# phoenix163/JeicybooDSP

Measured on AMD Instinct MI355X. Metric: STFT frames/s (1024-pt, 50% OLA), higher is better.
Workload: dtype f32; 1 GPU; STFT analysis n_fft=1024 hop=512 Hamming, batch=65536 frames/GPU, int16 PCM in HBM -> complex64 full spectrum in HBM; frames_per_gpu=65536, parallelism=frame-sharded x1, no collective, launch=hipGraph replay of the K steps, pcm_buffers=6, pcm_bytes_total=402659328

## Files before the change

### jeicyboodsp_amd/csrc/fft_c2c_kernels.hip

```cpp
#include "jdsp_internal.h"

namespace jdsp {

__device__ __forceinline__ short bitrev16(int k, int bits, int n_fft)
{
    short walk = (short)k;
    short rev = walk;
    for (int i = 1; i < bits; i++) {
        walk = (short)(walk >> 1);
        rev = (short)(unsigned short)(((unsigned)(unsigned short)rev) << 1);
        rev = (short)(rev | (walk & 1));
    }
    return (short)(rev & (n_fft - 1));
}

__global__ void bitrev_table_kernel(short *table, int n_fft, int bits)
{
    const int k = blockIdx.x * blockDim.x + threadIdx.x;
    if (k < n_fft) table[k] = bitrev16(k, bits, n_fft);
}

__global__ __launch_bounds__(256) void fft_process_f64_kernel(const double2 *__restrict__ in, double2 *__restrict__ out,
                                                             int n_fft, int log2n, int forward,
                                                             const double2 *__restrict__ tw)
{
    extern __shared__ __attribute__((aligned(16))) char smem_raw[];
    double2 *x = reinterpret_cast<double2 *>(smem_raw);
    const double2 *src = in + (size_t)blockIdx.x * n_fft;
    double2 *dst = out + (size_t)blockIdx.x * n_fft;
    for (int k = threadIdx.x; k < n_fft; k += blockDim.x)
        x[(unsigned short)bitrev16(k, log2n, n_fft)] = src[k];
    __syncthreads();
    const int half_n = n_fft >> 1;
// ... 248 lines not shown
#pragma unroll
    for (int d = 0; d < 8; d++) {
        const cd zm = lds[512 - lane - 64 * d];
        const double2 w = wsp[64 * d];
        const cd e = {v[d].x + zm.x, v[d].y - zm.y};
        const cd o = {v[d].y + zm.y, zm.x - v[d].x};
        const cd p = cd_mul(o, cd{w.x, w.y});
        f64x2 lo = {0.5 * (e.x + p.x), 0.5 * (e.y + p.y)}, hi = {0.5 * (e.x - p.x), 0.5 * (e.y - p.y)};
        __builtin_nontemporal_store(lo, dst + 64 * d);
        __builtin_nontemporal_store(hi, dst + 64 * d + 512);
    }
    lds_fence_wave();
  }
}

__device__ __forceinline__ void cd_opaque(cd &a) { asm volatile("" : "+v"(a.x), "+v"(a.y)); }
__device__ __forceinline__ void cd_powers(const cd &b, cd (&p)[8])
{
    p[1] = b;
    p[2] = cd_mul(b, b);
    p[3] = cd_mul(p[2], b);
    p[4] = cd_mul(p[2], p[2]);
    p[5] = cd_mul(p[4], b);
    p[6] = cd_mul(p[3], p[3]);
    p[7] = cd_mul(p[4], p[3]);
}

#ifndef JDSP_F64_PLAIN_STORES
#define JDSP_F64_PLAIN_STORES 0
#endif
#ifndef JDSP_F64_LINEAR_MAP
#define JDSP_F64_LINEAR_MAP 1
#endif
template <bool DW, bool LOOP>
__global__ __launch_bounds__(64, (JDSP_F64_SWIZZLE && !LOOP) ? 5 : 4) void stft1024_f64_v2_kernel(const short *__restrict__ pcm, long n_frames, long hop,
                                                               const double *__restrict__ table,
                                                               const double2 *__restrict__ tw, double2 *__restrict__ out,
                                                               int run)
{
    constexpr bool SWZ = JDSP_F64_SWIZZLE && !LOOP;
    __shared__ __attribute__((aligned(16))) cd lds[SWZ ? 512 : kFft512Lds];
    const int lane = threadIdx.x;
#if JDSP_F64_LINEAR_MAP
    const long t0 = (long)blockIdx.x * run;
#else
    const long per_xcd = (gridDim.x + 7) >> 3;
    const long t0 = ((long)(blockIdx.x & 7) * per_xcd + (blockIdx.x >> 3)) * run;
#endif
    if (t0 >= n_frames) return;
    const long t1 = LOOP ? (t0 + run < n_frames ? t0 + run : n_frames) : t0 + 1;
    double2 win[8];
    {
        const double2 *wp = reinterpret_cast<const double2 *>(table) + lane;
#pragma unroll
        for (int r = 0; r < 8; r++) win[r] = wp[64 * r];
    }
    cd b1 = w512<false>(tw, lane), b2 = w512<false>(tw, 8 * (lane & 7));
    cd b3;
    {
        const double2 q = (reinterpret_cast<const double2 *>(table + 1024))[lane];
        b3 = {q.x, q.y};
    }
    unsigned int raw[8];
    short raw16[16];
    auto fetch = [&](long t) {
        const short *src = pcm + t * hop + 2 * lane;
        if (DW) {
#pragma unroll
            for (int r = 0; r < 8; r++) raw[r] = *reinterpret_cast<const unsigned int *>(src + 128 * r);
        } else {
#pragma unroll
            for (int r = 0; r < 8; r++) { raw16[2 * r] = src[128 * r]; raw16[2 * r + 1] = src[128 * r + 1]; }
        }
    };
    fetch(t0);
    unsigned int tk[8];
#pragma unroll
    for (int r = 0; r < 8; r++) tk[r] = raw[r];
#pragma unroll 1
    for (long t = t0; t < t1; t++) {
// ... 63 lines not shown
        for (int d = 0; d < 8; d++) lds[lane + 64 * d] = v[d];
        if constexpr (!SWZ) { if (lane == 0) lds[512] = v[0]; }
        lds_fence_wave();
        if (LOOP && DW && t + 1 < t1) {
#pragma unroll
            for (int r = 0; r < 8; r++) { tk[r] = raw[r]; asm volatile("" : "+v"(tk[r])); }
            __builtin_amdgcn_sched_barrier(0);
        }
        typedef double f64x2 __attribute__((ext_vector_type(2)));
        f64x2 *dst = reinterpret_cast<f64x2 *>(out + t * 1024 + lane);
        constexpr double c1 = 0.92387953251128675613, s1 = 0.38268343236508977173, h = 0.70710678118654752440;
        const cd w16[8] = {{1.0, 0.0}, {c1, -s1}, {h, -h}, {s1, -c1}, {0.0, -1.0}, {-s1, -c1}, {-h, -h}, {-c1, -s1}};
#pragma unroll
        for (int d = 0; d < 8; d++) {
            const cd zm = lds[SWZ ? ((512 - lane - 64 * d) & 511) : (512 - lane - 64 * d)];
            const cd w = d == 0 ? b3 : (d == 4 ? cd{b3.y, -b3.x} : cd_mul(b3, w16[d]));
            const cd e = {v[d].x + zm.x, v[d].y - zm.y};
            const cd o = {v[d].y + zm.y, zm.x - v[d].x};
            const cd pp = cd_mul(o, w);
            f64x2 lo = {0.5 * (e.x + pp.x), 0.5 * (e.y + pp.y)}, hi = {0.5 * (e.x - pp.x), 0.5 * (e.y - pp.y)};
#if JDSP_F64_PLAIN_STORES
            dst[64 * d] = lo;
            dst[64 * d + 512] = hi;
#else
            __builtin_nontemporal_store(lo, dst + 64 * d);
            __builtin_nontemporal_store(hi, dst + 64 * d + 512);
#endif
        }
        lds_fence_wave();
    }
}

int launch_stft1024_f64(hipStream_t stream, int n_cu, const short *pcm, long n_frames, long hop, const double *table,
                        const double2 *tw512, double2 *out, int variant, int fpw)
{
    if (n_frames <= 0) return 0;
    const long slots = 4096;
    const long run = fpw > 0 ? fpw : (variant == 1 ? (n_frames + slots - 1) / slots : 1);
    (void)n_cu;
    const long waves = (n_frames + run - 1) / run;
    const long grid = (waves + 7) / 8 * 8;
    if (variant == 1)
        hipLaunchKernelGGL(stft1024_f64_kernel, dim3((unsigned)grid), dim3(64), 0, stream, pcm, n_frames, hop, table, tw512,
                           out, (int)run);
    else {
        const bool dw = (((uintptr_t)pcm) & 3u) == 0 && (hop & 1) == 0;
#define JDSP_F64_LAUNCH(DW_, LOOP_) hipLaunchKernelGGL((stft1024_f64_v2_kernel<DW_, LOOP_>), dim3((unsigned)grid), dim3(64), 0, stream, pcm, \
                                                       n_frames, hop, table, tw512, out, (int)run)
        if (run > 1) { if (dw) JDSP_F64_LAUNCH(true, true); else JDSP_F64_LAUNCH(false, true); }
        else { if (dw) JDSP_F64_LAUNCH(true, false); else JDSP_F64_LAUNCH(false, false); }
#undef JDSP_F64_LAUNCH
    }
    return hipGetLastError() == hipSuccess ? 0 : -1;
}

void fill_stft1024_f64_table(double *t)
{
    const double PI = 3.141592;
    for (int i = 0; i < 1024; i++) t[i] = 0.54 - 0.46 * cos(2 * PI * i / (1024 - 1));
    const double two_pi = 6.283185307179586476925286766559;
    for (int m = 0; m < 512; m++) {
        const double a = -two_pi * (double)m / 1024.0;
        t[1024 + 2 * m] = cos(a);
        t[1024 + 2 * m + 1] = sin(a);
    }
}

int launch_fft_process_f64(hipStream_t stream, const double2 *in, double2 *out, int n_fft, int log2n, long batch,
                           int forward, const double2 *tw)
{
    if (batch <= 0) return 0;
    if (n_fft == 512 && (((uintptr_t)in | (uintptr_t)out) & 15u) == 0) {
        const long grid = (batch + 7) / 8 * 8;
        if (forward) hipLaunchKernelGGL(fft512_f64_kernel<false>, dim3((unsigned)grid), dim3(64), 0, stream, in, out, batch, tw);
        else hipLaunchKernelGGL(fft512_f64_kernel<true>, dim3((unsigned)grid), dim3(64), 0, stream, in, out, batch, tw);
        return hipGetLastError() == hipSuccess ? 0 : -1;
    }
    const size_t lds = sizeof(double2) * (size_t)n_fft;
    int threads = n_fft / 2 < 256 ? (n_fft / 2 < 64 ? 64 : n_fft / 2) : 256;
    if (lds > 64 * 1024) {
        hipError_t e = hipFuncSetAttribute((const void *)fft_process_f64_kernel,
                                           hipFuncAttributeMaxDynamicSharedMemorySize, (int)lds);
        if (e != hipSuccess) return -1;
    }
    hipLaunchKernelGGL(fft_process_f64_kernel, dim3((unsigned)batch), dim3(threads), lds, stream, in, out, n_fft, log2n,
                       forward, tw);
// ... 14 lines not shown
```

### jeicyboodsp_amd/csrc/jdsp_api.hip

```cpp
#include "jdsp_internal.h"

static std::string g_create_error;

namespace jdsp {

int fail(jdsp_ctx *ctx, int code, const char *what, hipError_t e)
{
    std::string msg = what ? what : "error";
    if (e != hipSuccess) {
        msg += ": ";
        msg += hipGetErrorString(e);
    }
    if (ctx) ctx->error = msg;
    else g_create_error = msg;
    return code;
}

static int ensure_stft1024_table_of(jdsp_ctx *ctx, DevBuf<float2> &table, int window_kind)
{
    return ensure_table(ctx, table, (size_t)stft1024_table_count(),
                        [window_kind](float2 *t) { fill_stft1024_table(t, window_kind); });
}

int ensure_stft1024_table(jdsp_ctx *ctx) { return ensure_stft1024_table_of(ctx, ctx->stft1024_table, 0); }

int ensure_stft1024_table_rect(jdsp_ctx *ctx) { return ensure_stft1024_table_of(ctx, ctx->stft1024_table_rect, 2); }

int ensure_vad_window(jdsp_ctx *ctx)
{
    return ensure_table(ctx, ctx->vad_w_hi, 512, [](double *w) {
        for (int i = 0; i < 512; i++) w[i] = (0.54 - 0.46 * cos(2 * 3.141592 * (512 + i) / (1024 - 1)));
    });
}
// ... 19 lines not shown

int jdsp_abi_version(void) { return JDSP_ABI_VERSION; }

int jdsp_create(int device, jdsp_ctx **out)
{
    if (!out) return fail(nullptr, JDSP_EINVAL, "jdsp_create: out is NULL");
    *out = nullptr;
    int count = 0;
    hipError_t e = hipGetDeviceCount(&count);
    if (e != hipSuccess || count <= 0)
        return fail(nullptr, JDSP_ENODEV, "jdsp_create: no HIP device (this library has no CPU fallback)", e);
    if (device < 0 || device >= count) return fail(nullptr, JDSP_ENODEV, "jdsp_create: device ordinal out of range");
    jdsp_ctx *ctx = new (std::nothrow) jdsp_ctx();
    if (!ctx) return fail(nullptr, JDSP_ENOMEM, "jdsp_create: out of host memory");
    ctx->device = device;
    hipDeviceProp_t prop;
    if ((e = hipSetDevice(device)) != hipSuccess || (e = hipGetDeviceProperties(&prop, device)) != hipSuccess) {
        delete ctx;
        return fail(nullptr, JDSP_EHIP, "jdsp_create: device query", e);
    }
    ctx->n_cu = prop.multiProcessorCount;
    ctx->hbm_bytes = prop.totalGlobalMem;
    snprintf(ctx->name, sizeof(ctx->name), "%s (%s)", prop.name, prop.gcnArchName);
    if (strncmp(prop.gcnArchName, "gfx950", 6) != 0) {
        std::string m = std::string("jdsp_create: device is ") + prop.gcnArchName + ", this library is built for gfx950 only";
        delete ctx;
        return fail(nullptr, JDSP_ENODEV, m.c_str());
    }
    if ((e = hipStreamCreateWithFlags(&ctx->own_stream, hipStreamNonBlocking)) != hipSuccess) {
        delete ctx;
        return fail(nullptr, JDSP_EHIP, "jdsp_create: hipStreamCreate", e);
    }
    ctx->stream = ctx->own_stream;
    *out = ctx;
    return JDSP_OK;
}

int jdsp_destroy(jdsp_ctx *ctx)
{
    if (!ctx) return JDSP_OK;
    (void)hipSetDevice(ctx->device);
    (void)hipStreamSynchronize(ctx->stream);
    const hipEvent_t events[] = {ctx->pipe_ev[0], ctx->pipe_ev[1], ctx->pipe_ev[2], ctx->pipe_ev[3],
                                 ctx->pipe_ev[4], ctx->pipe_ev[5], ctx->switch_ev};
    const hipStream_t streams[] = {ctx->pipe_in, ctx->pipe_out, ctx->own_stream};
    delete ctx;
    for (hipEvent_t ev : events)
        if (ev) (void)hipEventDestroy(ev);
    for (hipStream_t st : streams)
        if (st) (void)hipStreamDestroy(st);
    return JDSP_OK;
}

const char *jdsp_last_error(const jdsp_ctx *ctx) { return ctx ? ctx->error.c_str() : g_create_error.c_str(); }

static int switch_stream(jdsp_ctx *ctx, hipStream_t next)
{
    if (next == ctx->stream) return JDSP_OK;
    hipStreamCaptureStatus a = hipStreamCaptureStatusNone, b = hipStreamCaptureStatusNone;
    const bool ok_a = hipStreamIsCapturing(ctx->stream, &a) == hipSuccess;
    const bool ok_b = hipStreamIsCapturing(next, &b) == hipSuccess;
    if (!ok_a || !ok_b) (void)hipGetLastError();
    if (ok_a && ok_b && a == hipStreamCaptureStatusNone && b == hipStreamCaptureStatusNone) {
        JDSP_HIP(ctx, hipSetDevice(ctx->device));
        if (!ctx->switch_ev) JDSP_HIP(ctx, hipEventCreateWithFlags(&ctx->switch_ev, hipEventDisableTiming));
        JDSP_HIP(ctx, hipEventRecord(ctx->switch_ev, ctx->stream));
// ... 239 lines not shown
    float *d_max = hc.alloc<float>(n * 4);
    float *d_ac = autocorr_host ? hc.alloc<float>(n * 2048) : nullptr;
    if (hc.ok()) hc.result(jdsp_pitch_autocorr_dev(ctx, d_in, n_blocks, d_prev, d_arg, d_max, d_ac));
    hc.download(arg_host, d_arg, n * 4);
    hc.download(rmax_host, d_max, n * 4);
    hc.download(autocorr_host, d_ac, n * 2048);
    return hc.finish();
}

int jdsp_stft_i16_dev(jdsp_ctx *ctx, const int16_t *pcm_dev, long n_frames, int n_fft, int hop, jdsp_c32 *spec_dev)
{
    if (!ctx) return JDSP_EINVAL;
    if (n_fft != 1024 && n_fft != 512) return fail(ctx, JDSP_EINVAL, "jdsp_stft_i16_dev: n_fft must be 1024 or 512");
    if (hop < 1) return fail(ctx, JDSP_EINVAL, "jdsp_stft_i16_dev: hop must be >= 1");
    if (n_frames < 0 || (n_frames > 0 && (!pcm_dev || !spec_dev)))
        return fail(ctx, JDSP_EINVAL, "jdsp_stft_i16_dev: bad buffer");
    if (n_frames == 0) return JDSP_OK;
    if ((uintptr_t)pcm_dev & 1u) return fail(ctx, JDSP_EINVAL, "jdsp_stft_i16_dev: pcm must be 2-byte aligned");
    if ((uintptr_t)spec_dev & 15u) return fail(ctx, JDSP_EINVAL, "jdsp_stft_i16_dev: spec must be 16-byte aligned");
    JDSP_HIP(ctx, hipSetDevice(ctx->device));
    int rc = jdsp::ensure_stft1024_table(ctx);
    if (rc) return rc;
    const int wk = ctx->opt_stft_window;
    if (wk == 1 && (rc = jdsp::ensure_stft1024_table_of(ctx, ctx->stft1024_table_hann, 1))) return rc;
    const float2 *tab = wk == 1 ? ctx->stft1024_table_hann.get() : ctx->stft1024_table.get();
    if (n_fft == 512) {
        jdsp::DevBuf<float2> &w512 = wk == 1 ? ctx->win512_hann : ctx->win512;
        if ((rc = jdsp::ensure_table(ctx, w512, 256, [wk](float2 *w) { jdsp::fill_win512(w, wk); }))) return rc;
        if (jdsp::launch_stft512(ctx->stream, ctx->n_cu, pcm_dev, n_frames, hop, (float2 *)spec_dev, tab, w512.get()))
            return fail(ctx, JDSP_EHIP, "stft512 launch", hipGetLastError());
        return JDSP_OK;
    }
    if (jdsp::launch_stft1024(ctx->stream, ctx->n_cu, ctx->opt_stft_fpw, pcm_dev, n_frames, hop, (float2 *)spec_dev, tab,
                              ctx->opt_stft_read_pass, ctx->opt_stft_touch_wg))
        return fail(ctx, JDSP_EHIP, "stft1024 launch", hipGetLastError());
    return JDSP_OK;
}

int jdsp_stft_half_i16_dev(jdsp_ctx *ctx, const int16_t *pcm_dev, long n_frames, jdsp_c32 *spec_dev, long row_pitch)
{
    if (!ctx) return JDSP_EINVAL;
    if (n_frames < 0 || (n_frames > 0 && (!pcm_dev || !spec_dev))) return fail(ctx, JDSP_EINVAL, "jdsp_stft_half_i16_dev: bad buffer");
    if (row_pitch < 513) return fail(ctx, JDSP_EINVAL, "jdsp_stft_half_i16_dev: row_pitch must be at least 513");
    if (n_frames == 0) return JDSP_OK;
    if (((uintptr_t)pcm_dev & 15u) || ((uintptr_t)spec_dev & 15u))
        return fail(ctx, JDSP_EINVAL, "jdsp_stft_half_i16_dev: buffers must be 16-byte aligned");
    JDSP_HIP(ctx, hipSetDevice(ctx->device));
    int rc = jdsp::ensure_stft1024_table(ctx);
    if (rc) return rc;
    if (jdsp::launch_stft1024_half(ctx->stream, pcm_dev, n_frames, (float2 *)spec_dev, row_pitch, ctx->stft1024_table.get()))
        return fail(ctx, JDSP_EHIP, "stft half launch", hipGetLastError());
    return JDSP_OK;
}

static const char kStftBatchPitch[] =
    "jdsp_stft_half_batch: row_pitch must be even and >= 514 (every row 16-byte aligned: the even-row store)";

int jdsp_stft_half_batch_dev(jdsp_ctx *ctx, const int16_t *pcm_dev, const int64_t *sample_first_dev,
                             const int64_t *frame_first_dev, long n_utts, long n_frames_total, int hop, jdsp_c32 *spec_dev,
                             long row_pitch)
{
    if (!ctx) return JDSP_EINVAL;
    if (n_utts < 0 || n_frames_total < 0) return fail(ctx, JDSP_EINVAL, "jdsp_stft_half_batch: n_utts or n_frames_total < 0");
    if (hop != 1024 && hop != 512 && hop != 256)
        return fail(ctx, JDSP_EINVAL, "jdsp_stft_half_batch: hop must be 1024, 512 or 256 (n_fft, n_fft/2 or n_fft/4)");
    if (row_pitch < 514 || (row_pitch & 1)) return fail(ctx, JDSP_EINVAL, kStftBatchPitch);
    if (!jdsp::aligned(pcm_dev, 4) || !jdsp::aligned(spec_dev, 16) || !jdsp::aligned(sample_first_dev, 8) ||
// ... 62 lines not shown
        e = hipEventRecord(ev_comp[b], comp);
        if (e == hipSuccess) e = hipStreamWaitEvent(ctx->pipe_out, ev_comp[b], 0);
        if (e == hipSuccess) e = hipMemcpyAsync(spec_host + (size_t)f0 * n_fft, d_out, sizeof(jdsp_c32) * (size_t)nf * n_fft, hipMemcpyDeviceToHost, ctx->pipe_out);
        if (e == hipSuccess) e = hipEventRecord(ev_out[b], ctx->pipe_out);
        if (e != hipSuccess) rc = fail(ctx, JDSP_EHIP, "stft pipeline: copy out", e);
    }
    hipError_t e1 = hipStreamSynchronize(ctx->pipe_in), e2 = hipStreamSynchronize(comp), e3 = hipStreamSynchronize(ctx->pipe_out);
    if (!rc && (e1 != hipSuccess || e2 != hipSuccess || e3 != hipSuccess)) rc = fail(ctx, JDSP_EHIP, "stft pipeline: sync", e1 != hipSuccess ? e1 : (e2 != hipSuccess ? e2 : e3));
    return rc;
}

static int ensure_c2c_tw(jdsp_ctx *ctx, int n_fft, int lg)
{
    return jdsp::ensure_table(ctx, ctx->c2c_tw[lg], (size_t)n_fft / 2 + 1,
                              [n_fft](double2 *t) { jdsp::fill_c2c_twiddles(t, n_fft); });
}

int jdsp_stft_i16_f64_dev(jdsp_ctx *ctx, const int16_t *pcm_dev, long n_frames, int n_fft, int hop, double *spec_dev)
{
    if (!ctx) return JDSP_EINVAL;
    if (n_fft != 1024) return fail(ctx, JDSP_EINVAL, "jdsp_stft_i16_f64_dev: n_fft must be 1024");
    if (hop < 1) return fail(ctx, JDSP_EINVAL, "jdsp_stft_i16_f64_dev: hop must be >= 1");
    if (n_frames < 0 || (n_frames > 0 && (!pcm_dev || !spec_dev))) return fail(ctx, JDSP_EINVAL, "jdsp_stft_i16_f64_dev: bad buffer");
    if (n_frames == 0) return JDSP_OK;
    if ((uintptr_t)pcm_dev & 1u) return fail(ctx, JDSP_EINVAL, "jdsp_stft_i16_f64_dev: pcm must be 2-byte aligned");
    if ((uintptr_t)spec_dev & 15u) return fail(ctx, JDSP_EINVAL, "jdsp_stft_i16_f64_dev: spec must be 16-byte aligned");
    JDSP_HIP(ctx, hipSetDevice(ctx->device));
    int rc = ensure_c2c_tw(ctx, 512, 9);
    if (rc) return rc;
    if ((rc = jdsp::ensure_table(ctx, ctx->stft_f64_table, 1024 + 2 * 512, jdsp::fill_stft1024_f64_table))) return rc;
    const int rp = ctx->opt_stft_read_pass;
    const bool touch = hop == 512 && ((uintptr_t)pcm_dev & 15u) == 0 && (rp > 0 || (rp < 0 && n_frames >= 16384));
    const long slab = touch ? 65536 : n_frames;
    for (long f0 = 0; f0 < n_frames; f0 += slab) {
        const long nf = n_frames - f0 < slab ? n_frames - f0 : slab;
        if ((touch && jdsp::launch_pcm_read_pass(ctx->stream, ctx->n_cu, ctx->opt_stft_touch_wg, pcm_dev + f0 * hop, hop * (nf + 1))) ||
            jdsp::launch_stft1024_f64(ctx->stream, ctx->n_cu, pcm_dev + f0 * hop, nf, hop, ctx->stft_f64_table.get(), ctx->c2c_tw[9].get(),
                                      (double2 *)spec_dev + f0 * 1024, ctx->opt_stft_f64_kernel, ctx->opt_stft_f64_fpw)) {
            const hipError_t le = hipGetLastError();
            return fail(ctx, JDSP_EHIP, "stft f64 launch", le);
        }
    }
    return JDSP_OK;
}

int jdsp_stft_i16_f64(jdsp_ctx *ctx, const int16_t *pcm_host, long n_samples, int n_fft, int hop, double *spec_host,
                      long *n_frames_out)
{
    if (!ctx) return JDSP_EINVAL;
    if (n_fft != 1024 || hop < 1) return fail(ctx, JDSP_EINVAL, "jdsp_stft_i16_f64: unsupported n_fft/hop");
    const long n_frames = n_samples >= n_fft ? (n_samples - n_fft) / hop + 1 : 0;
    if (n_frames_out) *n_frames_out = n_frames;
    if (n_frames == 0) return JDSP_OK;
    if (!pcm_host || !spec_host) return fail(ctx, JDSP_EINVAL, "jdsp_stft_i16_f64: NULL buffer");
    JDSP_HIP(ctx, hipSetDevice(ctx->device));
    const size_t in_bytes = sizeof(int16_t) * (size_t)((n_frames - 1) * hop + n_fft);
    const size_t out_bytes = 2 * sizeof(double) * (size_t)n_frames * (size_t)n_fft;
    jdsp::HostCall hc(ctx, "jdsp_stft_i16_f64");
    const int16_t *d_in = hc.upload(pcm_host, in_bytes);
    double *d_out = hc.alloc<double>(out_bytes);
    if (hc.ok()) hc.result(jdsp_stft_i16_f64_dev(ctx, d_in, n_frames, n_fft, hop, d_out));
    hc.download(spec_host, d_out, out_bytes);
    return hc.finish();
}

int jdsp_stft_i16(jdsp_ctx *ctx, const int16_t *pcm_host, long n_samples, int n_fft, int hop, jdsp_c32 *spec_host,
                  long *n_frames_out)
{
    if (!ctx) return JDSP_EINVAL;
    if ((n_fft != 1024 && n_fft != 512) || hop < 1) return fail(ctx, JDSP_EINVAL, "jdsp_stft_i16: unsupported n_fft/hop");
    long n_frames = n_samples >= n_fft ? (n_samples - n_fft) / hop + 1 : 0;
// ... 51 lines not shown
```

### jeicyboodsp_amd/csrc/jdsp_internal.h

```cpp
#pragma once
#include <hip/hip_runtime.h>

#include <cmath>
#include <cstdlib>
#include <cstdint>
#include <cstdio>
#include <cstring>
#include <string>
#include <vector>

#include "../../include/jdsp.h"
#include "ragged_layout.h"

namespace jdsp {

template <class T> class DevBuf {
public:
    DevBuf() = default;
    DevBuf(DevBuf &&o) noexcept : p_(o.p_), n_(o.n_) { o.p_ = nullptr, o.n_ = 0; }
    DevBuf &operator=(DevBuf &&o) noexcept
    {
        if (this != &o) {
            reset();
            p_ = o.p_, n_ = o.n_;
// ... 16 lines not shown
        void *p = nullptr;
        const hipError_t e = hipMalloc(&p, count * sizeof(T));
        if (e == hipSuccess) p_ = (T *)p, n_ = count;
        return e;
    }
    hipError_t upload(const T *host, size_t count)
    {
        hipError_t e = alloc(count);
        if (e == hipSuccess && (e = hipMemcpy(p_, host, count * sizeof(T), hipMemcpyHostToDevice)) != hipSuccess) reset();
        return e;
    }
    hipError_t grow(size_t count) { return count <= n_ ? hipSuccess : alloc(count); }

private:
    T *p_ = nullptr;
    size_t n_ = 0;
};

}

struct jdsp_ctx {
    int device = 0;
    int n_cu = 0;
    size_t hbm_bytes = 0;
    char name[64] = {0};
    hipStream_t own_stream = nullptr;
    hipStream_t stream = nullptr;
    hipEvent_t switch_ev = nullptr;
    std::string error;
    int opt_stft_fpw = 0;
    int opt_stft_window = 0;
    int opt_stft_read_pass = -1;
    int opt_stft_touch_wg = 0;
    int opt_stft_f64_kernel = 0;
    int opt_stft_f64_fpw = 0;
    jdsp::DevBuf<float2> stft1024_table;
    jdsp::DevBuf<float2> stft1024_table_hann, win512_hann;
    jdsp::DevBuf<float2> stft1024_table_rect;
    jdsp::DevBuf<float2> win512;
    jdsp::DevBuf<double2> c2c_tw[16];
    jdsp::DevBuf<double> stft_f64_table;
    jdsp::DevBuf<float2> conv_tw4096, conv_tw8192;
    jdsp::DevBuf<double> vad_w_hi;
    jdsp::DevBuf<double> vad_w_ex[2][2];
    jdsp::DevBuf<double> lpc_win[2];
    hipStream_t pipe_in = nullptr, pipe_out = nullptr;
    hipEvent_t pipe_ev[6] = {nullptr, nullptr, nullptr, nullptr, nullptr, nullptr};
    jdsp::DevBuf<char> pipe_buf[4];
};

namespace jdsp {

struct DenoiseState {
    int run_len;
    int pad[3];
    float avg[1024];
    float noise[1024];
    short prev[512];
    float tail[512];
};
struct DenoisePlan { int n_events, n_snap, pad0, pad1; };

constexpr int kNoiseChunks = 4096;
struct NoiseAccum {
    float *chunk_alpha;
    float *chunk_beta;
// ... 143 lines not shown

template <class T, class Fill> int ensure_table(jdsp_ctx *ctx, DevBuf<T> &buf, size_t count, Fill fill)
{
    if (buf.get()) return JDSP_OK;
    std::vector<T> host(count);
    fill(host.data());
    const hipError_t e = buf.upload(host.data(), count);
    return e == hipSuccess ? JDSP_OK : fail(ctx, JDSP_EHIP, "device table", e);
}

struct RunPlanWs {
    DevBuf<unsigned char> flags;
    DevBuf<int> events, ev_n;
    DevBuf<int> ver_base;
    DevBuf<unsigned long long> snap_mask;
    long cap_blocks = 0;

    hipError_t reserve(size_t n)
    {
        hipError_t e = flags.alloc(n);
        if (e == hipSuccess) e = events.alloc(n);
        if (e == hipSuccess) e = ev_n.alloc(n);
        if (e == hipSuccess) e = ver_base.alloc(n / 64 + 1);
        if (e == hipSuccess) e = snap_mask.alloc(n / 64 + 1);
        if (e == hipSuccess) cap_blocks = (long)n;
        else *this = RunPlanWs();
        return e;
    }
};

int stft1024_table_count();
void fill_stft1024_table(float2 *host_table, int window_kind);
int launch_stft1024(hipStream_t stream, int n_cu, int fpw_opt, const short *pcm, long n_frames, long hop, float2 *spec,
                    const float2 *table, int read_pass = 0, int touch_wg_per_cu = 0);


int launch_stft1024_half(hipStream_t stream, const short *pcm, long n_frames, float2 *spec, long pitch,
                         const float2 *table);
int launch_stft512(hipStream_t stream, int n_cu, const short *pcm, long n_frames, long hop, float2 *spec,
                   const float2 *table, const float2 *win512);
void fill_win512(float2 *w, int window_kind);
int launch_stft_half_batch(hipStream_t s, int hop, int run_opt, const short *pcm, const long long *sample_first,
                           const long long *frame_first, long n_utts, long n_frames_total, float2 *spec, long pitch,
                           const float2 *table);

int launch_bitrev_table(hipStream_t stream, short *table_dev, int n_fft, int bits);
int launch_fft_process_f64(hipStream_t stream, const double2 *in, double2 *out, int n_fft, int log2n, long batch,
                           int forward, const double2 *tw);
void fill_c2c_twiddles(double2 *t, int n_fft);
int launch_stft1024_f64(hipStream_t stream, int n_cu, const short *pcm, long n_frames, long hop, const double *table,
                        const double2 *tw512, double2 *out, int variant, int fpw);
int launch_pcm_read_pass(hipStream_t stream, int n_cu, int wg_per_cu, const short *pcm, long n_samples);
void fill_stft1024_f64_table(double *t);
int launch_dft_direct_f64(hipStream_t stream, int kind, const void *in, double2 *inout, int n, long batch);


int launch_vad(hipStream_t s, int block_len, const short *pcm, long n_blocks, const double *w_hi, int use_zcr,
               unsigned char *flags, long long *dbg_energy, int *dbg_zcr);
int launch_run_plan(hipStream_t s, const unsigned char *flags, long n_blocks, const int *run_len_in, int *run_len_out,
                    int latch_run, int *ver_base, unsigned long long *snap_mask, int *events, int *ev_n,
                    DenoisePlan *plan);
int launch_denoise_plan(hipStream_t s, const unsigned char *flags, long n_blocks, const DenoiseState *st_in,
                        DenoiseState *st_out, int *ver_base, unsigned long long *snap_mask, int *events, int *ev_n,
                        DenoisePlan *plan);
int launch_noise_estimate(hipStream_t s, DenoiseGeom g, const short *pcm, long n_blocks, const DenoiseState *st_in,
                          DenoiseState *st_out, const int *events, const int *ev_n, const DenoisePlan *plan,
                          const int *ver_base, const unsigned long long *snap_mask, const float2 *table,
                          const NoiseAccum &acc, float *noise_rows);
int launch_denoise(hipStream_t s, DenoiseGeom g, int mode, int k_opt, int n_cu, const short *pcm, long n_blocks,
                   long calls_before, const DenoiseState *st_in, DenoiseState *st_out, const int *ver_base,
                   const unsigned long long *snap_mask, const float *noise_rows, const float2 *table, short *out,
                   float *precast, int *redo, const DenoiseShard *shard = nullptr);
int launch_shard_summary(hipStream_t s, DenoiseGeom g, const short *pcm_ext, long n_ext, long ext0, long b0, long b1,
                         const int *events, const int *ev_n, const DenoisePlan *plan, const int *ver_base,
                         const unsigned long long *snap_mask, const float2 *table, int *range, const NoiseAccum &acc,
                         float *rows, float *summary);
int launch_shard_rows(hipStream_t s, DenoiseGeom g, const float *summaries_all, int rank, long b0, long b1,
                      const DenoisePlan *plan, const int *range, const NoiseAccum &acc, float *a_in, float *rows,
                      float *last);
int launch_shard_row0(hipStream_t s, DenoiseGeom g, const float *last_all, int rank, float *rows);
int launch_denoise_batch(hipStream_t s, int mode, int run_opt, int n_cu, const short *pcm, const long long *sample_first,
                         const long long *block_first, long n_utts, long n_blocks, const double *w_hi,
                         const float2 *table, unsigned char *flags, int *row_idx, float *rows, int *redo, short *out,
                         float *precast, float *noise_last, int vad_only);
// ... 348 lines not shown
```

### jeicyboodsp_amd/csrc/stft_kernels.hip

```cpp
#include "frame_io.h"
#include "jdsp_internal.h"
#include "ola_stream.h"
#include "ragged_batch.h"

namespace jdsp {

#ifndef JDSP_STFT_K
#define JDSP_STFT_K 2
#endif
#ifndef JDSP_STFT_MINWAVES
#define JDSP_STFT_MINWAVES 4
#endif
#ifndef JDSP_STFT_XCD
#define JDSP_STFT_XCD 1
#endif
#ifndef JDSP_STFT_NT_LOAD
#define JDSP_STFT_NT_LOAD 0
#endif
#ifndef JDSP_STFT_NT
#define JDSP_STFT_NT 1
#endif
#ifndef JDSP_STFT_DIRECT
#define JDSP_STFT_DIRECT 1
#endif
#ifndef JDSP_STFT_ABLATE
#define JDSP_STFT_ABLATE 0
#endif

__device__ __forceinline__ void store_spec(float4 *p, float4 v)
{
#if JDSP_STFT_NT
    f32x4 t = {v.x, v.y, v.z, v.w};
    __builtin_nontemporal_store(t, reinterpret_cast<f32x4 *>(p));
#else
    *p = v;
#endif
}

template <int J>
__device__ __forceinline__ void split_store_j(const float2 *lds, int lane, const float2 *wsp, float4 *dst)
{
    const int m = 128 * J + 2 * lane;
    const float4 zz = *reinterpret_cast<const float4 *>(&lds[m]);
    float2 zr0, zr1;
    load_mirror_pair(lds, m, zr0, zr1);
    float2 lo0, hi0, lo1, hi1;
    split_fwd<J>(make_float2(zz.x, zz.y), zr0, wsp[0], lo0, hi0);
    split_fwd<J>(make_float2(zz.z, zz.w), zr1, wsp[1], lo1, hi1);
    store_spec(dst + 64 * J, make_float4(lo0.x, lo0.y, lo1.x, lo1.y));
    store_spec(dst + 64 * J + 256, make_float4(hi0.x, hi0.y, hi1.x, hi1.y));
}

__device__ __forceinline__ void split_and_store(const float2 *lds, int lane, const float2 *wsp, float2 *out_frame)
{
    float4 *dst = reinterpret_cast<float4 *>(out_frame) + lane;
    split_store_j<0>(lds, lane, wsp, dst);
    split_store_j<1>(lds, lane, wsp, dst);
    split_store_j<2>(lds, lane, wsp, dst);
    split_store_j<3>(lds, lane, wsp, dst);
}

template <int K>
__global__ __launch_bounds__(64, JDSP_STFT_MINWAVES) void stft1024_hop512_kernel(
    const short *__restrict__ pcm, float2 *__restrict__ spec, long n_frames, const float2 *__restrict__ table)
{
    __shared__ __attribute__((aligned(16))) float2 lds[kWaveLdsComplex];
    __shared__ __attribute__((aligned(16))) unsigned int stage[256];
    const int lane = threadIdx.x;
#if JDSP_STFT_XCD
    const long per_xcd = (gridDim.x + 7) >> 3;
    const long f0 = ((long)(blockIdx.x & 7) * per_xcd + (blockIdx.x >> 3)) * K;
#else
    const long f0 = (long)blockIdx.x * K;
#endif
    if (f0 >= n_frames) return;

#if JDSP_STFT_DIRECT
    const unsigned int *pcm32 = reinterpret_cast<const unsigned int *>(pcm) + lane;
    unsigned int half[K + 1][4];
#pragma unroll
    for (int h = 0; h <= K; h++) {
        const long hh = f0 + h <= n_frames ? f0 + h : n_frames;
#pragma unroll
        for (int q = 0; q < 4; q++) half[h][q] = pcm32[hh * 256 + 64 * q];
    }
#else
    const u32x4 *pcm128 = reinterpret_cast<const u32x4 *>(pcm) + lane;
    u32x4 half[K + 1];
#pragma unroll
    for (int h = 0; h <= K; h++) {
        const long hh = f0 + h <= n_frames ? f0 + h : n_frames;
#if JDSP_STFT_NT_LOAD
        half[h] = __builtin_nontemporal_load(pcm128 + hh * 64);
#else
        half[h] = pcm128[hh * 64];
#endif
    }
#endif

    FrameTables t;
    load_frame_tables(t, table, lane);

    unsigned int raw[8];
#if JDSP_STFT_DIRECT
#pragma unroll
    for (int q = 0; q < 4; q++) raw[4 + q] = half[0][q];
// ... 278 lines not shown
        store_natural_image(lds, lane, v);
        wave_lds_fence();
        float2 *dst = spec + f * 512;
        split_store_even_j<0>(lds, lane, wsp0, dst);
        split_store_even_j<1>(lds, lane, wsp0, dst);
        split_store_even_j<2>(lds, lane, wsp0, dst);
        split_store_even_j<3>(lds, lane, wsp0, dst);
        wave_lds_fence();
    }
}

int launch_stft512(hipStream_t stream, int n_cu, const short *pcm, long n_frames, long hop, float2 *spec,
                   const float2 *table, const float2 *win512)
{
    if (n_frames <= 0) return 0;
    const long fpw = n_frames >= 2L * n_cu * 16 ? 2 : 1;
    const long grid = (n_frames + fpw - 1) / fpw;
    hipLaunchKernelGGL(stft512_kernel, dim3((unsigned)grid), dim3(64), 0, stream, pcm, spec, n_frames, (int)fpw, hop,
                       table, win512);
    return hipGetLastError() == hipSuccess ? 0 : -1;
}

void fill_win512(float2 *w, int window_kind)
{
    const double wa = window_kind == 1 ? 0.5 : 0.54, wb = window_kind == 1 ? 0.5 : 0.46;
    for (int i = 0; i < 256; i++) {
        const double w0 = (wa - wb * cos(2 * 3.141592 * (2 * i) / (512 - 1)));
        const double w1 = (wa - wb * cos(2 * 3.141592 * (2 * i + 1) / (512 - 1)));
        w[i] = make_float2((float)(0.5 * w0), (float)(0.5 * w1));
    }
}

template <int K>
static void launch_hop512(hipStream_t stream, const short *pcm, long n_frames, float2 *spec, const float2 *table)
{
    long grid = (n_frames + K - 1) / K;
#if JDSP_STFT_XCD
    grid = (grid + 7) / 8 * 8;
#endif
    hipLaunchKernelGGL(stft1024_hop512_kernel<K>, dim3((unsigned)grid), dim3(64), 0, stream, pcm, spec, n_frames,
                       table);
}

constexpr long kReadPassSlabFrames = 65536;
constexpr long kReadPassMinFrames = 16384;

__global__ __launch_bounds__(256) void pcm_touch_kernel(const u32x4 *__restrict__ p, long n16, unsigned int *__restrict__ sink)
{
    const long stride = (long)gridDim.x * 256;
    long i = (long)blockIdx.x * 256 + threadIdx.x;
    unsigned int acc = 0;
    for (; i + 3 * stride < n16; i += 4 * stride) {
        const u32x4 a = p[i], b = p[i + stride], c = p[i + 2 * stride], d = p[i + 3 * stride];
        acc ^= a.x ^ b.x ^ c.x ^ d.x;
    }
    for (; i < n16; i += stride) acc ^= p[i].x;
    if (sink && acc == 0x9e3779b9u) *sink = acc;
}

static int launch_pcm_touch(hipStream_t stream, int n_cu, int wg_per_cu, const short *pcm, long n_samples)
{
    const long n16 = n_samples / 8;
    if (n16 <= 0) return 0;
    long grid = (long)n_cu * (wg_per_cu > 0 ? wg_per_cu : 4);
    const long need = (n16 + 255) / 256;
    if (grid > need) grid = need;
    hipLaunchKernelGGL(pcm_touch_kernel, dim3((unsigned)grid), dim3(256), 0, stream, reinterpret_cast<const u32x4 *>(pcm), n16,
                       (unsigned int *)nullptr);
    return hipGetLastError() == hipSuccess ? 0 : -1;
}

int launch_pcm_read_pass(hipStream_t stream, int n_cu, int wg_per_cu, const short *pcm, long n_samples)
{
    return launch_pcm_touch(stream, n_cu, wg_per_cu, pcm, n_samples);
}

static void launch_hop512_any(hipStream_t stream, int fpw_opt, const short *pcm, long n_frames, float2 *spec,
                              const float2 *table)
{
    switch (fpw_opt) {
    case 1: launch_hop512<1>(stream, pcm, n_frames, spec, table); break;
    case 2: launch_hop512<2>(stream, pcm, n_frames, spec, table); break;
    case 3: launch_hop512<3>(stream, pcm, n_frames, spec, table); break;
    case 4: launch_hop512<4>(stream, pcm, n_frames, spec, table); break;
    default: launch_hop512<JDSP_STFT_K>(stream, pcm, n_frames, spec, table); break;
    }
}

int launch_stft1024(hipStream_t stream, int n_cu, int fpw_opt, const short *pcm, long n_frames, long hop,
                    float2 *spec, const float2 *table, int read_pass, int touch_wg_per_cu)
{
    if (n_frames <= 0) return 0;
    if (hop == 512 && ((uintptr_t)pcm & 15u) == 0) {
        const bool touch = read_pass > 0 || (read_pass < 0 && n_frames >= kReadPassMinFrames);
#ifdef JDSP_PROBE_READ_PASS_ALONE
        if (read_pass == 1) {
            for (long f0 = 0; f0 < n_frames; f0 += kReadPassSlabFrames) {
                const long nf = n_frames - f0 < kReadPassSlabFrames ? n_frames - f0 : kReadPassSlabFrames;
                if (launch_pcm_touch(stream, n_cu, touch_wg_per_cu, pcm + f0 * 512, 512 * (nf + 1))) return -1;
            }
            return hipGetLastError() == hipSuccess ? 0 : -1;
        }
#endif
        if (!touch) {
            launch_hop512_any(stream, fpw_opt, pcm, n_frames, spec, table);
        } else {
            for (long f0 = 0; f0 < n_frames; f0 += kReadPassSlabFrames) {
                const long nf = n_frames - f0 < kReadPassSlabFrames ? n_frames - f0 : kReadPassSlabFrames;
                if (launch_pcm_touch(stream, n_cu, touch_wg_per_cu, pcm + f0 * 512, 512 * (nf + 1))) return -1;
                launch_hop512_any(stream, fpw_opt > 0 ? fpw_opt : 1, pcm + f0 * 512, nf, spec + f0 * 1024, table);
            }
        }
    } else {
        const long fpw = n_frames >= 2L * n_cu * 16 ? 2 : 1;
        long grid = (n_frames + fpw - 1) / fpw;
        hipLaunchKernelGGL(stft1024_anyhop_kernel, dim3((unsigned)grid), dim3(64), 0, stream, pcm, spec, n_frames,
                           (int)fpw, hop, table);
    }
    return hipGetLastError() == hipSuccess ? 0 : -1;
}

int stft1024_table_count() { return kStftTableCount; }

void fill_stft1024_table(float2 *t, int window_kind)
{
    const double wa = window_kind == 2 ? 1.0 : (window_kind == 1 ? 0.5 : 0.54);
    const double wb = window_kind == 2 ? 0.0 : (window_kind == 1 ? 0.5 : 0.46);
    const double two_pi = 6.283185307179586476925286766559;
    for (int k = 1; k < 8; k++)
        for (int l = 0; l < 64; l++) {
            double a = -two_pi * (double)(l * k) / 512.0;
            t[kTwT1 + (k - 1) * 64 + l] = make_float2((float)cos(a), (float)sin(a));
        }
    for (int c = 1; c < 8; c++)
        for (int b = 0; b < 8; b++) {
            double a = -two_pi * (double)(b * c) / 64.0;
            t[kTwT2 + (c - 1) * 8 + b] = make_float2((float)cos(a), (float)sin(a));
        }
    for (int i = 0; i < 512; i++) {
        double w0 = (wa - wb * cos(2 * 3.141592 * (2 * i) / (1024 - 1)));
        double w1 = (wa - wb * cos(2 * 3.141592 * (2 * i + 1) / (1024 - 1)));
        t[kStftWin + i] = make_float2((float)(0.5 * w0), (float)(0.5 * w1));
        t[kStftWinFull + i] = make_float2((float)w0, (float)w1);
// ... 9 lines not shown
```

Measured before the change: 649.8 million frames/s.

## Fuse PCM read-pass touch into STFT kernel launch as leading touch blocks

The separate pcm_touch prefetch kernel that ran before each STFT slab is folded into the STFT kernel itself. The first touch_blocks workgroups stream the PCM slab to warm the cache, and the remaining blocks do the STFT with remapped block indices. The touch block count is derived from an occupancy query made at context creation. This removes one launch and the kernel boundary per slab, so touching can overlap with compute, but the touch blocks now share the grid with FFT blocks and may contend with them for CUs and bandwidth.

```diff
diff --git a/jeicyboodsp_amd/csrc/fft_c2c_kernels.hip b/jeicyboodsp_amd/csrc/fft_c2c_kernels.hip
--- a/jeicyboodsp_amd/csrc/fft_c2c_kernels.hip
+++ b/jeicyboodsp_amd/csrc/fft_c2c_kernels.hip
@@ -1,4 +1,5 @@
 #include "jdsp_internal.h"
+#include "pcm_touch.h"
 
 namespace jdsp {
 
@@ -313,20 +314,30 @@
 #ifndef JDSP_F64_LINEAR_MAP
 #define JDSP_F64_LINEAR_MAP 1
 #endif
-template <bool DW, bool LOOP>
+template <bool DW, bool LOOP, bool TOUCH>
 __global__ __launch_bounds__(64, (JDSP_F64_SWIZZLE && !LOOP) ? 5 : 4) void stft1024_f64_v2_kernel(const short *__restrict__ pcm, long n_frames, long hop,
                                                                const double *__restrict__ table,
                                                                const double2 *__restrict__ tw, double2 *__restrict__ out,
-                                                               int run)
+                                                               int run, unsigned int touch_blocks, unsigned int *__restrict__ sink)
 {
     constexpr bool SWZ = JDSP_F64_SWIZZLE && !LOOP;
     __shared__ __attribute__((aligned(16))) cd lds[SWZ ? 512 : kFft512Lds];
     const int lane = threadIdx.x;
+    unsigned int block = blockIdx.x, blocks = gridDim.x;
+    if constexpr (TOUCH) {
+        if (block < touch_blocks) {
+            pcm_touch_role(reinterpret_cast<const u32x4 *>(pcm), 64 * (n_frames + 1), block, touch_blocks, lane, sink);
+            return;
+        }
+        block -= touch_blocks;
+        blocks -= touch_blocks;
+    }
 #if JDSP_F64_LINEAR_MAP
-    const long t0 = (long)blockIdx.x * run;
+    (void)blocks;
+    const long t0 = (long)block * run;
 #else
-    const long per_xcd = (gridDim.x + 7) >> 3;
-    const long t0 = ((long)(blockIdx.x & 7) * per_xcd + (blockIdx.x >> 3)) * run;
+    const long per_xcd = (blocks + 7) >> 3;
+    const long t0 = ((long)(block & 7) * per_xcd + (block >> 3)) * run;
 #endif
     if (t0 >= n_frames) return;
     const long t1 = LOOP ? (t0 + run < n_frames ? t0 + run : n_frames) : t0 + 1;
@@ -456,9 +467,10 @@
 }
 
 int launch_stft1024_f64(hipStream_t stream, int n_cu, const short *pcm, long n_frames, long hop, const double *table,
-                        const double2 *tw512, double2 *out, int variant, int fpw)
+                        const double2 *tw512, double2 *out, int variant, int fpw, long touch_blocks)
 {
     if (n_frames <= 0) return 0;
+    if (touch_blocks > 0 && (variant != 0 || fpw > 1 || hop != 512 || (((uintptr_t)pcm) & 15u) || (touch_blocks & 7))) return -1;
     const long slots = 4096;
     const long run = fpw > 0 ? fpw : (variant == 1 ? (n_frames + slots - 1) / slots : 1);
     (void)n_cu;
@@ -469,13 +481,22 @@
                            out, (int)run);
     else {
         const bool dw = (((uintptr_t)pcm) & 3u) == 0 && (hop & 1) == 0;
-#define JDSP_F64_LAUNCH(DW_, LOOP_) hipLaunchKernelGGL((stft1024_f64_v2_kernel<DW_, LOOP_>), dim3((unsigned)grid), dim3(64), 0, stream, pcm, \
-                                                       n_frames, hop, table, tw512, out, (int)run)
-        if (run > 1) { if (dw) JDSP_F64_LAUNCH(true, true); else JDSP_F64_LAUNCH(false, true); }
+#define JDSP_F64_LAUNCH(DW_, LOOP_) hipLaunchKernelGGL((stft1024_f64_v2_kernel<DW_, LOOP_, false>), dim3((unsigned)grid), dim3(64), 0, stream, pcm, \
+                                                       n_frames, hop, table, tw512, out, (int)run, 0u, (unsigned int *)nullptr)
+        if (touch_blocks > 0)
+            hipLaunchKernelGGL((stft1024_f64_v2_kernel<true, false, true>), dim3((unsigned)(touch_blocks + grid)), dim3(64), 0, stream,
+                               pcm, n_frames, hop, table, tw512, out, (int)run, (unsigned int)touch_blocks, (unsigned int *)nullptr);
+        else if (run > 1) { if (dw) JDSP_F64_LAUNCH(true, true); else JDSP_F64_LAUNCH(false, true); }
         else { if (dw) JDSP_F64_LAUNCH(true, false); else JDSP_F64_LAUNCH(false, false); }
 #undef JDSP_F64_LAUNCH
     }
     return hipGetLastError() == hipSuccess ? 0 : -1;
+}
+
+int stft_f64_resident_blocks(int *out)
+{
+    const hipError_t e = hipOccupancyMaxActiveBlocksPerMultiprocessor(out, stft1024_f64_v2_kernel<true, false, true>, 64, 0);
+    return e == hipSuccess && *out > 0 ? 0 : -1;
 }
 
 void fill_stft1024_f64_table(double *t)
diff --git a/jeicyboodsp_amd/csrc/jdsp_api.hip b/jeicyboodsp_amd/csrc/jdsp_api.hip
--- a/jeicyboodsp_amd/csrc/jdsp_api.hip
+++ b/jeicyboodsp_amd/csrc/jdsp_api.hip
@@ -1,4 +1,5 @@
 #include "jdsp_internal.h"
+#include "pcm_touch.h"
 
 static std::string g_create_error;
 
@@ -84,6 +85,12 @@
         return fail(nullptr, JDSP_EHIP, "jdsp_create: hipStreamCreate", e);
     }
     ctx->stream = ctx->own_stream;
+    if (jdsp::stft_hop512_resident_blocks(ctx->stft_resident) || jdsp::stft_f64_resident_blocks(&ctx->stft_f64_resident)) {
+        e = hipGetLastError();
+        (void)hipStreamDestroy(ctx->own_stream);
+        delete ctx;
+        return fail(nullptr, JDSP_EHIP, "jdsp_create: occupancy query of the STFT analysis kernels", e);
+    }
     *out = ctx;
     return JDSP_OK;
 }
@@ -389,7 +396,7 @@
         return JDSP_OK;
     }
     if (jdsp::launch_stft1024(ctx->stream, ctx->n_cu, ctx->opt_stft_fpw, pcm_dev, n_frames, hop, (float2 *)spec_dev, tab,
-                              ctx->opt_stft_read_pass, ctx->opt_stft_touch_wg))
+                              ctx->opt_stft_read_pass, ctx->opt_stft_touch_wg, ctx->stft_resident))
         return fail(ctx, JDSP_EHIP, "stft1024 launch", hipGetLastError());
     return JDSP_OK;
 }
@@ -518,11 +525,17 @@
     const int rp = ctx->opt_stft_read_pass;
     const bool touch = hop == 512 && ((uintptr_t)pcm_dev & 15u) == 0 && (rp > 0 || (rp < 0 && n_frames >= 16384));
     const long slab = touch ? 65536 : n_frames;
+#if defined(JDSP_STFT_TWO_LAUNCH) && JDSP_STFT_TWO_LAUNCH
+    const bool fused = false;
+#else
+    const bool fused = touch && ctx->opt_stft_f64_kernel == 0 && ctx->opt_stft_f64_fpw <= 1;
+#endif
     for (long f0 = 0; f0 < n_frames; f0 += slab) {
         const long nf = n_frames - f0 < slab ? n_frames - f0 : slab;
-        if ((touch && jdsp::launch_pcm_read_pass(ctx->stream, ctx->n_cu, ctx->opt_stft_touch_wg, pcm_dev + f0 * hop, hop * (nf + 1))) ||
+        const long g = fused ? jdsp::stft_touch_blocks(ctx->n_cu, ctx->opt_stft_touch_wg, ctx->stft_f64_resident, 64 * (nf + 1)) : 0;
+        if ((touch && !fused && jdsp::launch_pcm_read_pass(ctx->stream, ctx->n_cu, ctx->opt_stft_touch_wg, pcm_dev + f0 * hop, hop * (nf + 1))) ||
             jdsp::launch_stft1024_f64(ctx->stream, ctx->n_cu, pcm_dev + f0 * hop, nf, hop, ctx->stft_f64_table.get(), ctx->c2c_tw[9].get(),
-                                      (double2 *)spec_dev + f0 * 1024, ctx->opt_stft_f64_kernel, ctx->opt_stft_f64_fpw)) {
+                                      (double2 *)spec_dev + f0 * 1024, ctx->opt_stft_f64_kernel, ctx->opt_stft_f64_fpw, g)) {
             const hipError_t le = hipGetLastError();
             return fail(ctx, JDSP_EHIP, "stft f64 launch", le);
         }
diff --git a/jeicyboodsp_amd/csrc/jdsp_internal.h b/jeicyboodsp_amd/csrc/jdsp_internal.h
--- a/jeicyboodsp_amd/csrc/jdsp_internal.h
+++ b/jeicyboodsp_amd/csrc/jdsp_internal.h
@@ -72,6 +72,8 @@
     int opt_stft_window = 0;
     int opt_stft_read_pass = -1;
     int opt_stft_touch_wg = 0;
+    int stft_resident[5] = {0, 0, 0, 0, 0};
+    int stft_f64_resident = 0;
     int opt_stft_f64_kernel = 0;
     int opt_stft_f64_fpw = 0;
     jdsp::DevBuf<float2> stft1024_table;
@@ -281,7 +283,8 @@
 int stft1024_table_count();
 void fill_stft1024_table(float2 *host_table, int window_kind);
 int launch_stft1024(hipStream_t stream, int n_cu, int fpw_opt, const short *pcm, long n_frames, long hop, float2 *spec,
-                    const float2 *table, int read_pass = 0, int touch_wg_per_cu = 0);
+                    const float2 *table, int read_pass = 0, int touch_wg_per_cu = 0, const int *touch_resident = nullptr);
+int stft_hop512_resident_blocks(int out[5]);
 
 
 int launch_stft1024_half(hipStream_t stream, const short *pcm, long n_frames, float2 *spec, long pitch,
@@ -298,7 +301,8 @@
                            int forward, const double2 *tw);
 void fill_c2c_twiddles(double2 *t, int n_fft);
 int launch_stft1024_f64(hipStream_t stream, int n_cu, const short *pcm, long n_frames, long hop, const double *table,
-                        const double2 *tw512, double2 *out, int variant, int fpw);
+                        const double2 *tw512, double2 *out, int variant, int fpw, long touch_blocks = 0);
+int stft_f64_resident_blocks(int *out);
 int launch_pcm_read_pass(hipStream_t stream, int n_cu, int wg_per_cu, const short *pcm, long n_samples);
 void fill_stft1024_f64_table(double *t);
 int launch_dft_direct_f64(hipStream_t stream, int kind, const void *in, double2 *inout, int n, long batch);
diff --git a/jeicyboodsp_amd/csrc/pcm_touch.h b/jeicyboodsp_amd/csrc/pcm_touch.h
--- /dev/null
+++ b/jeicyboodsp_amd/csrc/pcm_touch.h
@@ -0,0 +1,30 @@
+#pragma once
+#include <hip/hip_runtime.h>
+
+#include "frame_io.h"
+
+namespace jdsp {
+
+__device__ __forceinline__ void pcm_touch_role(const u32x4 *__restrict__ p, long n16, long b, long blocks, int lane,
+                                               unsigned int *__restrict__ sink)
+{
+    const long stride = blocks * 64;
+    long i = b * 64 + lane;
+    unsigned int acc = 0;
+    for (; i + 3 * stride < n16; i += 4 * stride) {
+        const u32x4 a0 = p[i], a1 = p[i + stride], a2 = p[i + 2 * stride], a3 = p[i + 3 * stride];
+        acc ^= a0.x ^ a1.x ^ a2.x ^ a3.x;
+    }
+    for (; i < n16; i += stride) acc ^= p[i].x;
+    if (sink && acc == 0x9e3779b9u) *sink = acc;
+}
+
+inline long stft_touch_blocks(int n_cu, int per_cu, int resident, long n16)
+{
+    long g = (long)n_cu * (per_cu > 0 ? per_cu : resident);
+    const long need = (n16 + 63) / 64;
+    if (g > need) g = need;
+    return (g + 7) / 8 * 8;
+}
+
+}
diff --git a/jeicyboodsp_amd/csrc/stft_kernels.hip b/jeicyboodsp_amd/csrc/stft_kernels.hip
--- a/jeicyboodsp_amd/csrc/stft_kernels.hip
+++ b/jeicyboodsp_amd/csrc/stft_kernels.hip
@@ -1,6 +1,7 @@
 #include "frame_io.h"
 #include "jdsp_internal.h"
 #include "ola_stream.h"
+#include "pcm_touch.h"
 #include "ragged_batch.h"
 
 namespace jdsp {
@@ -22,6 +23,9 @@
 #endif
 #ifndef JDSP_STFT_DIRECT
 #define JDSP_STFT_DIRECT 1
+#endif
+#ifndef JDSP_STFT_TWO_LAUNCH
+#define JDSP_STFT_TWO_LAUNCH 0
 #endif
 #ifndef JDSP_STFT_ABLATE
 #define JDSP_STFT_ABLATE 0
@@ -60,18 +64,28 @@
     split_store_j<3>(lds, lane, wsp, dst);
 }
 
-template <int K>
+template <int K, bool TOUCH>
 __global__ __launch_bounds__(64, JDSP_STFT_MINWAVES) void stft1024_hop512_kernel(
-    const short *__restrict__ pcm, float2 *__restrict__ spec, long n_frames, const float2 *__restrict__ table)
+    const short *__restrict__ pcm, float2 *__restrict__ spec, long n_frames, const float2 *__restrict__ table,
+    unsigned int touch_blocks, unsigned int *__restrict__ sink)
 {
     __shared__ __attribute__((aligned(16))) float2 lds[kWaveLdsComplex];
     __shared__ __attribute__((aligned(16))) unsigned int stage[256];
     const int lane = threadIdx.x;
+    unsigned int block = blockIdx.x, blocks = gridDim.x;
+    if constexpr (TOUCH) {
+        if (block < touch_blocks) {
+            pcm_touch_role(reinterpret_cast<const u32x4 *>(pcm), 64 * (n_frames + 1), block, touch_blocks, lane, sink);
+            return;
+        }
+        block -= touch_blocks;
+        blocks -= touch_blocks;
+    }
 #if JDSP_STFT_XCD
-    const long per_xcd = (gridDim.x + 7) >> 3;
-    const long f0 = ((long)(blockIdx.x & 7) * per_xcd + (blockIdx.x >> 3)) * K;
-#else
-    const long f0 = (long)blockIdx.x * K;
+    const long per_xcd = (blocks + 7) >> 3;
+    const long f0 = ((long)(block & 7) * per_xcd + (block >> 3)) * K;
+#else
+    const long f0 = (long)block * K;
 #endif
     if (f0 >= n_frames) return;
 
@@ -416,14 +430,19 @@
 }
 
 template <int K>
-static void launch_hop512(hipStream_t stream, const short *pcm, long n_frames, float2 *spec, const float2 *table)
+static void launch_hop512(hipStream_t stream, const short *pcm, long n_frames, float2 *spec, const float2 *table,
+                          long touch_blocks = 0)
 {
     long grid = (n_frames + K - 1) / K;
 #if JDSP_STFT_XCD
     grid = (grid + 7) / 8 * 8;
 #endif
-    hipLaunchKernelGGL(stft1024_hop512_kernel<K>, dim3((unsigned)grid), dim3(64), 0, stream, pcm, spec, n_frames,
-                       table);
+    if (touch_blocks > 0)
+        hipLaunchKernelGGL((stft1024_hop512_kernel<K, true>), dim3((unsigned)(touch_blocks + grid)), dim3(64), 0, stream, pcm,
+                           spec, n_frames, table, (unsigned int)touch_blocks, (unsigned int *)nullptr);
+    else
+        hipLaunchKernelGGL((stft1024_hop512_kernel<K, false>), dim3((unsigned)grid), dim3(64), 0, stream, pcm, spec, n_frames,
+                           table, 0u, (unsigned int *)nullptr);
 }
 
 constexpr long kReadPassSlabFrames = 65536;
@@ -460,19 +479,31 @@
 }
 
 static void launch_hop512_any(hipStream_t stream, int fpw_opt, const short *pcm, long n_frames, float2 *spec,
-                              const float2 *table)
+                              const float2 *table, long touch_blocks = 0)
 {
     switch (fpw_opt) {
-    case 1: launch_hop512<1>(stream, pcm, n_frames, spec, table); break;
-    case 2: launch_hop512<2>(stream, pcm, n_frames, spec, table); break;
-    case 3: launch_hop512<3>(stream, pcm, n_frames, spec, table); break;
-    case 4: launch_hop512<4>(stream, pcm, n_frames, spec, table); break;
-    default: launch_hop512<JDSP_STFT_K>(stream, pcm, n_frames, spec, table); break;
-    }
+    case 1: launch_hop512<1>(stream, pcm, n_frames, spec, table, touch_blocks); break;
+    case 2: launch_hop512<2>(stream, pcm, n_frames, spec, table, touch_blocks); break;
+    case 3: launch_hop512<3>(stream, pcm, n_frames, spec, table, touch_blocks); break;
+    case 4: launch_hop512<4>(stream, pcm, n_frames, spec, table, touch_blocks); break;
+    default: launch_hop512<JDSP_STFT_K>(stream, pcm, n_frames, spec, table, touch_blocks); break;
+    }
+}
+
+int stft_hop512_resident_blocks(int out[5])
+{
+    hipError_t e = hipOccupancyMaxActiveBlocksPerMultiprocessor(&out[0], stft1024_hop512_kernel<JDSP_STFT_K, true>, 64, 0);
+    if (e == hipSuccess) e = hipOccupancyMaxActiveBlocksPerMultiprocessor(&out[1], stft1024_hop512_kernel<1, true>, 64, 0);
+    if (e == hipSuccess) e = hipOccupancyMaxActiveBlocksPerMultiprocessor(&out[2], stft1024_hop512_kernel<2, true>, 64, 0);
+    if (e == hipSuccess) e = hipOccupancyMaxActiveBlocksPerMultiprocessor(&out[3], stft1024_hop512_kernel<3, true>, 64, 0);
+    if (e == hipSuccess) e = hipOccupancyMaxActiveBlocksPerMultiprocessor(&out[4], stft1024_hop512_kernel<4, true>, 64, 0);
+    for (int k = 0; k <= 4 && e == hipSuccess; k++)
+        if (out[k] <= 0) return -1;
+    return e == hipSuccess ? 0 : -1;
 }
 
 int launch_stft1024(hipStream_t stream, int n_cu, int fpw_opt, const short *pcm, long n_frames, long hop,
-                    float2 *spec, const float2 *table, int read_pass, int touch_wg_per_cu)
+                    float2 *spec, const float2 *table, int read_pass, int touch_wg_per_cu, const int *touch_resident)
 {
     if (n_frames <= 0) return 0;
     if (hop == 512 && ((uintptr_t)pcm & 15u) == 0) {
@@ -489,10 +520,17 @@
         if (!touch) {
             launch_hop512_any(stream, fpw_opt, pcm, n_frames, spec, table);
         } else {
+            const int k = fpw_opt >= 1 && fpw_opt <= 4 ? fpw_opt : (fpw_opt > 0 ? JDSP_STFT_K : 1);
+            if (!touch_resident) return -1;
             for (long f0 = 0; f0 < n_frames; f0 += kReadPassSlabFrames) {
                 const long nf = n_frames - f0 < kReadPassSlabFrames ? n_frames - f0 : kReadPassSlabFrames;
+#if JDSP_STFT_TWO_LAUNCH
                 if (launch_pcm_touch(stream, n_cu, touch_wg_per_cu, pcm + f0 * 512, 512 * (nf + 1))) return -1;
-                launch_hop512_any(stream, fpw_opt > 0 ? fpw_opt : 1, pcm + f0 * 512, nf, spec + f0 * 1024, table);
+                launch_hop512_any(stream, k, pcm + f0 * 512, nf, spec + f0 * 1024, table);
+#else
+                launch_hop512_any(stream, k, pcm + f0 * 512, nf, spec + f0 * 1024, table,
+                                  stft_touch_blocks(n_cu, touch_wg_per_cu, touch_resident[fpw_opt > 4 ? 0 : k], 64 * (nf + 1)));
+#endif
             }
         }
     } else {
```

Result: no change. 650.0 million frames/s (median of 2 runs) (+0.0%).
